# MDAnalysis/transport-analysis

Hardware: AMD Instinct MI355X
Metric: VACF lag-points/sec (n_frames x n_atoms / s) (higher is better)
Workload: dtype f64

## Files before the change

### transport_analysis_amd/csrc/wfft.hpp

```cpp
#pragma once
#include <hip/hip_runtime.h>

#include <type_traits>
#include <utility>

#include "fft_engine.hpp"

namespace ta {

#ifndef WF_NW_R0
#define WF_NW_R0 0
#define WF_NW_VAL 0
#endif

template <int LO, int HI, class F>
__device__ __forceinline__ void static_for_range(F&& f) {
    [&]<int... I>(std::integer_sequence<int, I...>) {
        (f(std::integral_constant<int, LO + I>{}), ...);
    }(std::make_integer_sequence<int, (HI > LO ? HI - LO : 0)>{});
}

typedef unsigned int wf_u32x4 __attribute__((ext_vector_type(4)));

#include "wfft_twist.inc"

template <>
struct Dft<3> {
    static __device__ __forceinline__ void run(cd (&v)[3]) {
        constexpr double kS3 = 0.86602540378443864676372317075294;
        const cd t = v[1] + v[2], d = v[1] - v[2];
        const cd m = cd{v[0].x - 0.5 * t.x, v[0].y - 0.5 * t.y};
        const cd e = cd{kS3 * d.y, -kS3 * d.x};
        v[0] = v[0] + t;
        v[1] = m + e;
        v[2] = m - e;
    }
};

template <int N>
struct DftOddTables;
template <>
struct DftOddTables<7> {
    static constexpr double c[3] = {0.62348980185873353053, -0.22252093395631440429, -0.90096886790241912624};
    static constexpr double s[3] = {0.78183148246802980871, 0.97492791218182360702, 0.43388373911755812048};
};
template <>
struct DftOddTables<9> {
    static constexpr double c[4] = {0.76604444311897803520, 0.17364817766693034885, -0.5, -0.93969262078590838405};
    static constexpr double s[4] = {0.64278760968653932632, 0.98480775301220805937, 0.86602540378443864676,
                                    0.34202014332566873304};
};
template <int N>
__device__ __forceinline__ void dft_odd(cd (&v)[N]) {
    constexpr int H = N / 2;
    using Tb = DftOddTables<N>;
    cd sp[H], dm[H];
#pragma unroll
    for (int j = 1; j <= H; ++j) {
        sp[j - 1] = v[j] + v[N - j];
        dm[j - 1] = v[j] - v[N - j];
    }
    const cd x0 = v[0];
    cd sum = x0;
#pragma unroll
    for (int j = 0; j < H; ++j) sum = sum + sp[j];
    v[0] = sum;
#pragma unroll
    for (int k = 1; k <= H; ++k) {
        double rx = x0.x, ry = x0.y, ix = 0.0, iy = 0.0;
#pragma unroll
        for (int j = 1; j <= H; ++j) {
            const int m = (j * k) % N;
            const double cm = m == 0 ? 1.0 : Tb::c[(m <= H ? m : N - m) - 1];
            const double sm = m == 0 ? 0.0 : m <= H ? Tb::s[m - 1] : -Tb::s[N - m - 1];
            rx = fma(cm, sp[j - 1].x, rx);
            ry = fma(cm, sp[j - 1].y, ry);
            ix = fma(sm, dm[j - 1].x, ix);
            iy = fma(sm, dm[j - 1].y, iy);
        }
        v[k] = cd{rx + iy, ry - ix};
        v[N - k] = cd{rx - iy, ry + ix};
    }
}
template <>
struct Dft<7> {
    static __device__ __forceinline__ void run(cd (&v)[7]) { dft_odd<7>(v); }
};
template <>
struct Dft<9> {
    static __device__ __forceinline__ void run(cd (&v)[9]) { dft_odd<9>(v); }
};

template <int N2>
__device__ __forceinline__ void dft_2x(cd (&v)[2 * N2]) {
    constexpr int N = 2 * N2;
    cd s[2][N2];
#pragma unroll
    for (int j2 = 0; j2 < N2; ++j2) {
        const cd a = v[(2 * j2) % N], b = v[(N2 + 2 * j2) % N];
        s[0][j2] = a + b;
        s[1][j2] = a - b;
    }
    Dft<N2>::run(s[0]);
    Dft<N2>::run(s[1]);
#pragma unroll
    for (int q = 0; q < N; ++q) v[q] = s[q % 2][q % N2];
}
template <>
struct Dft<14> {
    static __device__ __forceinline__ void run(cd (&v)[14]) { dft_2x<7>(v); }
};
template <>
struct Dft<18> {
    static __device__ __forceinline__ void run(cd (&v)[18]) { dft_2x<9>(v); }
};

template <>
struct Dft<6> {
    static __device__ __forceinline__ void run(cd (&v)[6]) {
        cd s[2][3];
#pragma unroll
        for (int j2 = 0; j2 < 3; ++j2) {
            const cd a = v[(2 * j2) % 6], b = v[(3 + 2 * j2) % 6];
            s[0][j2] = a + b;
            s[1][j2] = a - b;
        }
        Dft<3>::run(s[0]);
        Dft<3>::run(s[1]);
#pragma unroll
        for (int q = 0; q < 6; ++q) v[q] = s[q % 2][q % 3];
    }
};

template <>
struct Dft<12> {
    static __device__ __forceinline__ void run(cd (&v)[12]) {
        cd s[4][3];
#pragma unroll
        for (int j2 = 0; j2 < 3; ++j2) {
            cd t[4] = {v[(4 * j2) % 12], v[(3 + 4 * j2) % 12], v[(6 + 4 * j2) % 12], v[(9 + 4 * j2) % 12]};
            Dft<4>::run(t);
#pragma unroll
            for (int k1 = 0; k1 < 4; ++k1) s[k1][j2] = t[k1];
        }
#pragma unroll
        for (int k1 = 0; k1 < 4; ++k1) Dft<3>::run(s[k1]);
#pragma unroll
        for (int q = 0; q < 12; ++q) v[q] = s[q % 4][q % 3];
    }
};

template <>
struct Dft<10> {
    static __device__ __forceinline__ void run(cd (&v)[10]) {
        cd s[2][5];
#pragma unroll
        for (int j2 = 0; j2 < 5; ++j2) {
            const cd a = v[(2 * j2) % 10], b = v[(5 + 2 * j2) % 10];
            s[0][j2] = a + b;
            s[1][j2] = a - b;
        }
        Dft<5>::run(s[0]);
        Dft<5>::run(s[1]);
#pragma unroll
        for (int q = 0; q < 10; ++q) v[q] = s[q % 2][q % 5];
    }
};

template <>
struct Dft<20> {
    static __device__ __forceinline__ void run(cd (&v)[20]) {
        cd s[4][5];
#pragma unroll
        for (int j2 = 0; j2 < 5; ++j2) {
            cd t[4] = {v[(4 * j2) % 20], v[(5 + 4 * j2) % 20], v[(10 + 4 * j2) % 20], v[(15 + 4 * j2) % 20]};
            Dft<4>::run(t);
#pragma unroll
            for (int k1 = 0; k1 < 4; ++k1) s[k1][j2] = t[k1];
        }
#pragma unroll
        for (int k1 = 0; k1 < 4; ++k1) Dft<5>::run(s[k1]);
#pragma unroll
        for (int q = 0; q < 20; ++q) v[q] = s[q % 4][q % 5];
    }
};

template <int R0>
struct DftTwisted {
    static constexpr bool kHave = false;
};
template <int R0>
__device__ __forceinline__ cd wf_twist_in(const cd (&v)[R0], int n, int n2) {
    const cd x = v[n % R0];
    return ((n >= R0 ? 1 : 0) + n2) & 1 ? cd{-x.x, -x.y} : x;
}
template <>
struct DftTwisted<18> {
    static constexpr bool kHave = true;
    static __device__ __forceinline__ void run(cd (&v)[18]) {
        cd s[2][9];
#pragma unroll
        for (int j2 = 0; j2 < 9; ++j2) {
            const cd a = wf_twist_in<18>(v, 2 * j2, j2), b = wf_twist_in<18>(v, 9 + 2 * j2, j2);
            s[0][j2] = cd{a.x + b.y, a.y - b.x};
            s[1][j2] = cd{a.x - b.y, a.y + b.x};
        }
        Dft<9>::run(s[0]);
        Dft<9>::run(s[1]);
#pragma unroll
        for (int q = 0; q < 18; ++q) v[q] = s[q % 2][(q % 9 + 5) % 9];
    }
};
template <>
struct DftTwisted<20> {
    static constexpr bool kHave = true;
    static __device__ __forceinline__ void run(cd (&v)[20]) {
        cd s[4][5];
#pragma unroll
        for (int j2 = 0; j2 < 5; ++j2) {
            const cd a = wf_twist_in<20>(v, 4 * j2, j2), b = wf_twist_in<20>(v, 5 + 4 * j2, j2);
            const cd c = wf_twist_in<20>(v, 10 + 4 * j2, j2), d = wf_twist_in<20>(v, 15 + 4 * j2, j2);
            const cd p = cd{a.x + c.y, a.y - c.x}, m = cd{a.x - c.y, a.y + c.x};
            const cd e = cd{b.x + d.y, b.y - d.x}, f = cd{b.x - d.y, b.y + d.x};
            const double ex = e.x + e.y, ey = e.y - e.x;
            const double fx = f.y - f.x, fy = f.x + f.y;
            s[0][j2] = cd{fma(kR2, ex, p.x), fma(kR2, ey, p.y)};
            s[2][j2] = cd{fma(-kR2, ex, p.x), fma(-kR2, ey, p.y)};
            s[1][j2] = cd{fma(kR2, fx, m.x), fma(-kR2, fy, m.y)};
            s[3][j2] = cd{fma(-kR2, fx, m.x), fma(kR2, fy, m.y)};
        }
#pragma unroll
        for (int k1 = 0; k1 < 4; ++k1) Dft<5>::run(s[k1]);
#pragma unroll
        for (int q = 0; q < 20; ++q) v[q] = s[q % 4][(q % 5 + 3) % 5];
    }
};

constexpr int kWfStageRows = 14 + 8;
inline size_t wf_table_elems(int R0, int R) { return 2 * (size_t)R * R0 * 512 + kWfStageRows * 64; }
inline cd wf_tan_form(long num, long den) {
    const long double pi = 3.141592653589793238462643383279502884L;
    num %= den;
    if (4 * num == den) return cd{-0x1p200, 0x1p-200};
    if (4 * num == 3 * den) return cd{0x1p200, 0x1p-200};
    if (num == 0) return cd{0.0, 1.0};
    if (2 * num == den) return cd{0.0, -1.0};
    const long double h = 2.0L * pi * (long double)num / (long double)den;
    const long double c = cosl(h), sn = -sinl(h);
    return cd{(double)(sn / c), (double)c};
}
inline void wf_fill_table(int R0, int R, cd* a) {
    const long L = 2L * R * R0 * 512;
    const long double pi = 3.141592653589793238462643383279502884L;
    for (long n = 0; n < L; ++n) {
        if (n == 0) a[n] = cd{1.0, 0.0};
        else if (2 * n == L) a[n] = cd{-1.0, 0.0};
        else if (4 * n == L) a[n] = cd{0.0, -1.0};
        else if (4 * n == 3 * L) a[n] = cd{0.0, 1.0};
        else {
            const long double h = 2.0L * pi * (long double)n / (long double)L;
            a[n] = cd{(double)cosl(h), (double)-sinl(h)};
        }
    }
    for (int r = 1; r < 8; ++r)
        for (int l = 0; l < 64; ++l) {
            a[L + (r - 1) * 64 + l] = a[(L / 512) * l * r];
            a[L + (6 + r) * 64 + l] = a[(L / 64) * (l & 7) * r];
        }
    cd* t = a + L + 14 * 64;
    for (int l = 0; l < 64; ++l) {
        const long gb = 8 * (l >> 3), gc = 8 * (l & 7) + (l >> 3);
        const long g[2] = {gb, gc};
        for (int st = 0; st < 2; ++st) {
            t[(4 * st + 0) * 64 + l] = wf_tan_form(4 * g[st], 512);
            t[(4 * st + 1) * 64 + l] = wf_tan_form(2 * g[st], 512);
            t[(4 * st + 2) * 64 + l] = wf_tan_form(g[st], 512);
            t[(4 * st + 3) * 64 + l] = wf_tan_form(g[st] + 64, 512);
        }
    }
}

template <int R0_>
struct WPlan {
    static constexpr int R0 = R0_;
    static constexpr int N1 = 512;
    static constexpr int NW = R0 == WF_NW_R0 ? WF_NW_VAL : R0 <= 4 ? 2 : R0 <= 7 ? 4 : 8;
    static constexpr int NT = 64 * NW;
    static constexpr int K1 = (N1 + NT - 1) / NT;
#ifndef WF_SPREAD_ALL
    static constexpr bool kSpreadRows = R0 >= 9 && R0 <= 16;
#else
    static constexpr bool kSpreadRows = WF_SPREAD_ALL && (R0 < 18 || R0 == WF_NW_R0);
#endif
#ifndef WF_REG_EXCHANGE
    static constexpr bool kRegExchange = R0 >= 16;
#else
    static constexpr bool kRegExchange = WF_REG_EXCHANGE;
#endif
#ifndef WF_REG_EXCHANGE_SINGLE
    static constexpr bool kRegExchangeSingle = R0 == 2 || R0 == 7 || R0 == 9 || R0 == 10 || R0 == 12 || R0 == 14;
#else
    static constexpr bool kRegExchangeSingle = (WF_REG_EXCHANGE_SINGLE >> (R0 - 1)) & 1;
#endif
#ifndef WF_MINW_R0
    static __host__ __device__ constexpr int min_waves(bool , bool lng) { return R0 == 2 ? 4 : 1; }
#else
    static __host__ __device__ constexpr int min_waves(bool, bool) { return R0 == WF_MINW_R0 ? WF_MINW_VAL : 1; }
#endif
    static constexpr bool kTwResident = true;
    static constexpr int M = R0 * N1;
    static constexpr int NS1 = (R0 + NW - 1) / NW;
    static constexpr int NLO = R0 / NW, REM = R0 % NW;
    static __host__ __device__ constexpr int sub_count(int wave) { return NLO + (wave < REM ? 1 : 0); }
    static __host__ __device__ constexpr int sub_base(int wave) { return wave * NLO + (wave < REM ? wave : REM); }
    static constexpr size_t kLds = (size_t)M * sizeof(cd);

    struct RealSel {
        unsigned qmask[2];
        unsigned q1mask[2];
    };
    static __host__ __device__ constexpr int owner(int q) {
        for (int w = 0; w < NW; ++w)
            if (q >= sub_base(w) && q < sub_base(w) + sub_count(w)) return w;
        return 0;
    }
    static __host__ __device__ constexpr RealSel real_selection() {
        RealSel r{{0u, 0u}, {0u, 0u}};
        for (int t = 0; t < 2; ++t) {
            int load[8] = {0, 0, 0, 0, 0, 0, 0, 0}, simd[4] = {0, 0, 0, 0};
            auto take = [&](int q, bool self) {
                r.qmask[t] |= 1u << q;
                if (self) r.q1mask[t] |= 1u << q;
                ++load[owner(q)];
                ++simd[owner(q) % 4];
            };
            const int span = t == 0 ? R0 : R0 - 1;
            for (int q = 0; q < R0; ++q)
                if ((span - q + R0) % R0 == q) take(q, true);
            for (int q = 0; q < R0; ++q) {
                const int m = (span - q + R0) % R0;
                if (m <= q) continue;
                const int wa = owner(q), wb = owner(m);
                const int ca = 16 * load[wa] + simd[wa % 4], cb = 16 * load[wb] + simd[wb % 4];
                take(cb < ca ? m : q, false);
            }
        }
        return r;
    }
    static constexpr RealSel kRealSel = real_selection();
};

__device__ __forceinline__ cd wf_load(__amdgpu_buffer_rsrc_t r, unsigned lane_off, unsigned uni_off) {
    const wf_u32x4 v = __builtin_amdgcn_raw_buffer_load_b128(r, lane_off, uni_off, 0);
    return __builtin_bit_cast(cd, v);
}

struct WfSubPost {
    int lane, hi, lo;
    __device__ __forceinline__ explicit WfSubPost(int lane_) : lane(lane_) {
        asm volatile("" : "+v"(lane));
        hi = lane >> 3;
        lo = lane & 7;
    }
    __device__ __forceinline__ void read_a(const cd* __restrict__ reg, cd (&v)[8]) const {
#pragma unroll
        for (int n2 = 0; n2 < 8; ++n2) v[n2] = reg[64 * n2 + lane];
    }
    __device__ __forceinline__ void stage_a(cd* __restrict__ reg, cd (&v)[8], const cd (&twa)[7]) const {
        Dft<8>::run(v);
#pragma unroll
        for (int a = 1; a < 8; ++a) v[a] = cmul(v[a], twa[a - 1]);
        __builtin_amdgcn_wave_barrier();
#pragma unroll
        for (int a = 0; a < 8; ++a) reg[a * 64 + (lane ^ (8 * (a & 1)))] = v[a];
        __builtin_amdgcn_wave_barrier();
        const int base = hi * 64 + (lo ^ (8 * (hi & 1)));
#pragma unroll
        for (int n1 = 0; n1 < 8; ++n1) v[n1] = reg[base ^ (8 * n1)];
        __builtin_amdgcn_wave_barrier();
    }
    __device__ __forceinline__ void stage_b(cd* __restrict__ reg, cd (&v)[8], const cd (&twb)[7]) const {
        Dft<8>::run(v);
#pragma unroll
// ... 74 lines not shown
#pragma unroll
    for (int a = 0; a < 8; ++a)
        if (!(a & 1))
#pragma unroll
            for (int d = 0; d < 4; ++d) {
                const unsigned lo = w[a][d], hi = w[a | 1][d];
                w[a][d] = __builtin_amdgcn_update_dpp(lo, hi, 0x128, 0xF, 0xC, false);
                w[a | 1][d] = __builtin_amdgcn_update_dpp(hi, lo, 0x128, 0xF, 0x3, false);
            }
#pragma unroll
    for (int a = 0; a < 8; ++a) {
        wf_u32x4 t;
        t.x = w[a][0], t.y = w[a][1], t.z = w[a][2], t.w = w[a][3];
        v[a] = __builtin_bit_cast(cd, t);
    }
}

struct WfAddr {
    unsigned we, wo, re, ro, x16, b2w, b2r;
    __device__ __forceinline__ void init(int lane, unsigned q_bytes) {
        const int hi = lane >> 3, lo = lane & 7;
        we = q_bytes + 16u * (unsigned)lane;
        wo = q_bytes + 16u * (unsigned)(lane ^ 8);
        const unsigned rb = q_bytes + 16u * (unsigned)(hi * 64 + lo);
        re = rb + 128u * (unsigned)(hi & 1);
        ro = rb - 128u * (unsigned)(hi & 1);
        x16 = 16u * (unsigned)(hi ^ lo);
        b2w = q_bytes + 1024u * (unsigned)hi;
        b2r = b2w + 128u * (unsigned)lo;
    }
    __device__ __forceinline__ unsigned w2(int k) const { return (x16 ^ (16u * (unsigned)k)) + b2w; }
    __device__ __forceinline__ unsigned r2(int k) const { return (x16 ^ (16u * (unsigned)k)) + b2r; }
};
struct WfSub {
    const WfAddr& ad;
    unsigned char* smem;
    __device__ __forceinline__ WfSub(const WfAddr& ad_, unsigned char* smem_) : ad(ad_), smem(smem_) {}
    __device__ __forceinline__ cd& at(unsigned base, unsigned off) const {
        return *reinterpret_cast<cd*>(__builtin_assume_aligned(smem + (base + off), 16));
    }
    template <unsigned SO>
    __device__ __forceinline__ void read_a(cd (&v)[8]) const {
#pragma unroll
        for (int n2 = 0; n2 < 8; ++n2) v[n2] = at(ad.we, SO + 1024u * n2);
    }
    template <unsigned SO>
    __device__ __forceinline__ void stage_a_w(cd (&v)[8]) const {
        Dft<8>::run(v);
        __builtin_amdgcn_wave_barrier();
#pragma unroll
        for (int a = 0; a < 8; ++a) at(a & 1 ? ad.wo : ad.we, SO + 1024u * a) = v[a];
        __builtin_amdgcn_wave_barrier();
    }
    template <unsigned SO>
    __device__ __forceinline__ void stage_a_r(cd (&v)[8]) const {
        __builtin_amdgcn_wave_barrier();
#pragma unroll
        for (int n1 = 0; n1 < 8; ++n1) v[n1] = at(n1 & 1 ? ad.ro : ad.re, SO + 128u * n1);
        __builtin_amdgcn_wave_barrier();
    }
    template <unsigned SO, bool XV = false>
    __device__ __forceinline__ void stage_a(cd (&v)[8]) const {
        if constexpr (XV) {
            Dft<8>::run(v);
            wf_transpose_hi(v);
        } else {
            stage_a_w<SO>(v);
            stage_a_r<SO>(v);
        }
    }
    template <unsigned SO>
    __device__ __forceinline__ void stage_b_w(cd (&v)[8], const WfTw& tw) const {
        wf_dft8_tw(v, tw.b);
        __builtin_amdgcn_wave_barrier();
#pragma unroll
        for (int b = 0; b < 8; ++b) at(ad.w2(b), SO + 128u * b) = v[b];
        __builtin_amdgcn_wave_barrier();
    }
    template <unsigned SO>
    __device__ __forceinline__ void stage_b_r(cd (&v)[8]) const {
        __builtin_amdgcn_wave_barrier();
#pragma unroll
        for (int n0 = 0; n0 < 8; ++n0) v[n0] = at(ad.r2(n0), SO);
        __builtin_amdgcn_wave_barrier();
    }
    template <unsigned SO>
    __device__ __forceinline__ void stage_b(cd (&v)[8], const WfTw& tw) const {
        stage_b_w<SO>(v, tw);
        stage_b_r<SO>(v);
    }
    __device__ __forceinline__ void stage_c(cd (&v)[8], const WfTw& tw, double (&acc)[8]) const {
        wf_dft8_tw(v, tw.c);
#pragma unroll
        for (int c = 0; c < 8; ++c) acc[c] = fma(v[c].y, v[c].y, fma(v[c].x, v[c].x, acc[c]));
    }
    __device__ __forceinline__ void stage_c_w(cd (&v)[8], const WfTw& tw, double (&acc)[8], double wgt) const {
        wf_dft8_tw(v, tw.c);
#pragma unroll
        for (int c = 0; c < 8; ++c) acc[c] = fma(wgt, fma(v[c].y, v[c].y, v[c].x * v[c].x), acc[c]);
    }
};

constexpr unsigned kWfSubBytes = 512 * sizeof(cd);

struct WfNoHook {
    template <class T>
    __device__ __forceinline__ void operator()(T) const {}
};
template <int I>
using wf_part = std::integral_constant<int, I>;

template <int S0, bool XV = false, class Hook = WfNoHook>
__device__ __forceinline__ void wf_sub512(const WfSub& w, const WfTw& tw, double (&acc)[8], Hook&& hook = Hook{}) {
    cd v[8];
    w.read_a<S0 * kWfSubBytes>(v);
    hook(wf_part<0>{});
    w.template stage_a<S0 * kWfSubBytes, XV>(v);
    hook(wf_part<1>{});
    w.stage_b<S0 * kWfSubBytes>(v, tw);
    hook(wf_part<2>{});
    w.stage_c(v, tw, acc);
    hook(wf_part<3>{});
}

template <int S0, bool XV = false>
__device__ __forceinline__ void wf_sub512_w(const WfSub& w, const WfTw& tw, double (&acc)[8], double wgt) {
    cd v[8];
    w.read_a<S0 * kWfSubBytes>(v);
    w.template stage_a<S0 * kWfSubBytes, XV>(v);
    w.stage_b<S0 * kWfSubBytes>(v, tw);
    w.stage_c_w(v, tw, acc, wgt);
}

template <int S0, bool XV = false, class Hook = WfNoHook>
__device__ __forceinline__ void wf_sub512_x2(const WfSub& w, const WfTw& tw, double (&acc0)[8],
                                             double (&acc1)[8], Hook&& hook = Hook{}) {
    constexpr unsigned A = S0 * kWfSubBytes, B = A + kWfSubBytes;
    cd v0[8], v1[8];
    w.read_a<A>(v0);
    w.read_a<B>(v1);
    __builtin_amdgcn_wave_barrier();
    hook(wf_part<0>{});
    w.template stage_a<A>(v0);
    w.template stage_a<B, XV>(v1);
    hook(wf_part<1>{});
    w.stage_b<A>(v0, tw);
    w.stage_b<B>(v1, tw);
    hook(wf_part<2>{});
    w.stage_c(v0, tw, acc0);
    w.stage_c(v1, tw, acc1);
    hook(wf_part<3>{});
}

template <bool XV = false, class Hook = WfNoHook>
__device__ __forceinline__ void wf_sub512_x3(const WfSub& w, const WfTw& tw, double (&acc0)[8],
                                             double (&acc1)[8], double (&acc2)[8], Hook&& hook = Hook{}) {
    constexpr unsigned A = 0, B = kWfSubBytes, C = 2 * kWfSubBytes;
    cd v0[8], v1[8], v2[8];
    w.read_a<A>(v0);
    w.read_a<B>(v1);
    w.read_a<C>(v2);
    __builtin_amdgcn_wave_barrier();
    hook(wf_part<0>{});
    w.template stage_a<A>(v0);
    w.template stage_a<B>(v1);
    w.template stage_a<C, XV>(v2);
    hook(wf_part<1>{});
    w.stage_b<A>(v0, tw);
    w.stage_b<B>(v1, tw);
    w.stage_b<C>(v2, tw);
    hook(wf_part<2>{});
    w.stage_c(v0, tw, acc0);
    w.stage_c(v1, tw, acc1);
    w.stage_c(v2, tw, acc2);
    hook(wf_part<3>{});
}

__device__ __forceinline__ void wf_unit_of(long atom, int k, int D, long* pair, int* kind) {
    const long c0 = atom * D;
    if (D == 2) {
        *pair = atom, *kind = 2;
    } else if (D == 1) {
        *pair = c0 >> 1, *kind = (int)(c0 & 1);
    } else if ((c0 & 1) == 0) {
        *pair = (c0 >> 1) + k, *kind = k == 0 ? 2 : 0;
    } else {
        *pair = (c0 >> 1) + k, *kind = k == 0 ? 1 : 2;
    }
}

typedef unsigned int wf_u32x2 __attribute__((__vector_size__(2 * sizeof(unsigned int))));

__device__ __forceinline__ cd wf_cfma(cd acc, cd a, cd b) {
    return {acc.x + (a.x * b.x - a.y * b.y), acc.y + (a.x * b.y + a.y * b.x)};
}

template <bool S, class A, class B>
__device__ __forceinline__ auto& wf_pick(A& a, B& b) {
    if constexpr (S) return a;
    else return b;
}

#ifndef WF_PASS_SPLIT
#define WF_PASS_SPLIT 1
#endif
#ifndef WF_SEED_DERIVE
#define WF_SEED_DERIVE 2
#endif
#ifndef WF_TWIST_FOLD
#define WF_TWIST_FOLD 1
#endif
#ifndef WF_TWIDDLE_MIRROR
#define WF_TWIDDLE_MIRROR 1
#endif
template <class P, bool BYP, bool LONG, bool SRC32>
constexpr bool wf_pass_split = WF_PASS_SPLIT && !BYP && !LONG && !SRC32 && (P::R0 == 18 || P::R0 == 20);

__device__ __forceinline__ cd wf_csqr(cd a) { return {a.x * a.x - a.y * a.y, 2.0 * (a.x * a.y)}; }

template <class P, bool BYP, bool LONG, bool STAMP, bool SRC32, int PASS>
__device__ __forceinline__ void wf_accum_body(unsigned char* smem_raw, const double* __restrict__ pm, long pitch, int T,
                                              long n_units, const cd* __restrict__ tw2, double* __restrict__ accg, int D,
                                              int R_arg, unsigned long long* __restrict__ stamps) {
    cd* lds = reinterpret_cast<cd*>(smem_raw);
    constexpr int R0 = P::R0, N1 = P::N1, NW = P::NW, NS1 = P::NS1, M = P::M;
    static_assert(!(SRC32 && LONG), "float32 slabs: plans without an outer radix only");
    static_assert(PASS < 0 || (!BYP && !LONG), "a compile-time pass: lag sums without an outer radix");
    const int R = LONG ? R_arg : 1, npass = 2 * R, L = npass * M;
    const int tid = threadIdx.x, wave = tid >> 6;
    int lane = tid & 63;
    const int bi = blockIdx.x >> 3;
    const int pass = PASS >= 0 ? PASS : bi % npass;
    constexpr bool kTwistFold = PASS == 1 && WF_TWIST_FOLD && DftTwisted<R0>::kHave;
    constexpr bool kMirror = PASS >= 0 && WF_TWIDDLE_MIRROR && R0 % 2 == 0;
    const long tuple = (blockIdx.x & 7) + 8 * (bi / npass), n_tuples = gridDim.x / npass;
    const int upa = BYP ? (D == 3 ? 2 : 1) : 1;
    const int grp = BYP && (D & 1) ? 2 : 1;

    double acc[NS1][8];
#pragma unroll
    for (int s = 0; s < NS1; ++s)
#pragma unroll
        for (int c = 0; c < 8; ++c) acc[s][c] = 0.0;
    unsigned long long st_acc[4] = {0, 0, 0, 0}, st_prev = 0, st_t0 = 0, st_r0 = 0, st_tail = 0, st_s2end = 0;
    if constexpr (STAMP) {
        st_prev = st_t0 = __builtin_amdgcn_s_memtime();
        st_r0 = __builtin_amdgcn_s_memrealtime();
    }
#define WF_STAMP(i)                                                   \
    if constexpr (STAMP) {                                            \
        const unsigned long long now_ = __builtin_amdgcn_s_memtime(); \
        st_acc[i] += now_ - st_prev;                                  \
        st_prev = now_;                                               \
    }
    const __amdgpu_buffer_rsrc_t twr =
        __builtin_amdgcn_make_buffer_rsrc(const_cast<cd*>(tw2), 0, (L + kWfStageRows * 64) * 16, 0x00020000);
    auto unit_rsrc = [&](long item, int k, int* kind) {
        long pair = item;
        const bool live = item < n_units;
        *kind = 2;
        if constexpr (BYP) wf_unit_of(live ? item : 0, k, D, &pair, kind);
        if constexpr (SRC32)
            return __builtin_amdgcn_make_buffer_rsrc(
                const_cast<float*>(reinterpret_cast<const float*>(pm) + (live ? pair : 0) * pitch * 2), 0,
                live ? T * 8 : 0, 0x00020000);
        else
            return __builtin_amdgcn_make_buffer_rsrc(const_cast<double*>(pm + (live ? pair : 0) * pitch * 2), 0,
                                                     live ? T * 16 : 0, 0x00020000);
    };
    using RowT = std::conditional_t<SRC32, wf_u32x2, cd>;
    auto load_row = [&](__amdgpu_buffer_rsrc_t rs, int kd, int u, unsigned row_off) -> RowT {
        if constexpr (SRC32) {
            return __builtin_amdgcn_raw_buffer_load_b64(rs, (unsigned)u * 8u, row_off * 8u, 0);
        } else {
            if (!BYP || kd == 2) return wf_load(rs, (unsigned)u * 16u, row_off * 16u);
            return cd{__builtin_bit_cast(double, __builtin_amdgcn_raw_buffer_load_b64(
                                                     rs, (unsigned)u * 16u + (unsigned)kd * 8u, row_off * 16u, 0)),
                      0.0};
        }
    };
    [[maybe_unused]] auto wf_widen = [&](wf_u32x2 r, int kd) {
        if (!BYP || kd == 2)
            return cd{(double)__builtin_bit_cast(float, (unsigned)r[0]), (double)__builtin_bit_cast(float, (unsigned)r[1])};
        return cd{(double)__builtin_bit_cast(float, (unsigned)(kd ? r[1] : r[0])), 0.0};
    };
    constexpr int K1 = P::K1, NT = P::NT;
    RowT xx[K1][R0];
    auto issue_loads = [&](__amdgpu_buffer_rsrc_t rs, int kd) {
#pragma unroll
        for (int k1 = 0; k1 < K1; ++k1) {
            const int u = tid + NT * k1;
            if (K1 * NT != N1 && u >= N1) continue;
            if (!BYP || kd == 2) {
#pragma unroll
                for (int j = 0; j < R0; ++j) xx[k1][j] = load_row(rs, 2, u, (unsigned)(N1 * j));
            } else {
#pragma unroll
                for (int j = 0; j < R0; ++j) xx[k1][j] = load_row(rs, kd, u, (unsigned)(N1 * j));
            }
        }
    };
#ifndef WF_LOAD_PARTS
#define WF_LOAD_PARTS 4
#endif
    constexpr int NR = K1 * R0;
    constexpr bool kSpread = P::kSpreadRows || (SRC32 && R0 >= 18);
#ifndef WF_SPREAD32_TAIL
#define WF_SPREAD32_TAIL 0
#endif
    constexpr int NSPREAD = WF_LOAD_PARTS != 4 ? 0 : (kSpread ? (SRC32 && R0 >= 18 ? NR - WF_SPREAD32_TAIL : NR) : 0);
    auto issue_row = [&](auto ii, __amdgpu_buffer_rsrc_t rs, int kd) {
        constexpr int i = decltype(ii)::value, k1 = i / R0, j = i % R0;
        const int u = tid + NT * k1;
        if (K1 * NT != N1 && u >= N1) return;
        if (!BYP || kd == 2) xx[k1][j] = load_row(rs, 2, u, (unsigned)(N1 * j));
        else xx[k1][j] = load_row(rs, kd, u, (unsigned)(N1 * j));
    };
    auto issue_loads_part = [&](auto part_c, __amdgpu_buffer_rsrc_t rs, int kd) {
        constexpr int PART = decltype(part_c)::value;
        static_for_range<PART * NSPREAD / 4, (PART + 1) * NSPREAD / 4>([&](auto ii) { issue_row(ii, rs, kd); });
    };
    auto issue_loads_tail = [&](__amdgpu_buffer_rsrc_t rs, int kd) {
        static_for_range<NSPREAD, NR>([&](auto ii) { issue_row(ii, rs, kd); });
    };
    int kind = 2, nkind = 2;
    __amdgpu_buffer_rsrc_t crs = unit_rsrc(tuple * grp, 0, &kind);
    issue_loads(crs, kind);
    WfTw stw;
    auto load_stage_tw = [&]() {
#pragma unroll
        for (int a = 0; a < 4; ++a) {
            stw.b[a] = wf_load(twr, (unsigned)lane * 16u, (unsigned)(L + (14 + a) * 64) * 16u);
            stw.c[a] = wf_load(twr, (unsigned)lane * 16u, (unsigned)(L + (18 + a) * 64) * 16u);
        }
    };
    constexpr bool kTwRes = P::kTwResident && !(BYP && LONG && R0 >= 18);
    if constexpr (kTwRes) load_stage_tw();
    WfAddr wad;
    wad.init(lane, (unsigned)P::sub_base(wave) * kWfSubBytes);
    const WfSub wsub(wad, smem_raw);
    int k = 0;
    bool zero_pending = false;
    for (long item = tuple * grp; item < n_units;) {
#ifndef WF_REAL_S1_SKIP
#define WF_REAL_S1_SKIP 0
#endif
        const unsigned qsel = (WF_REAL_S1_SKIP && BYP && kind != 2) ? P::kRealSel.qmask[pass ? 1 : 0] : ~0u;
#pragma unroll
        for (int k1 = 0; k1 < K1; ++k1) {
        const int u = tid + NT * k1;
        if (K1 * NT != N1 && u >= N1) continue;
        [[maybe_unused]] cd xwide[SRC32 ? R0 : 1];
        if constexpr (SRC32) {
#pragma unroll
            for (int j = 0; j < R0; ++j) xwide[j] = wf_widen(xx[k1][j], kind);
        }
        cd(&x)[R0] = wf_pick<SRC32>(xwide, xx[k1]);
        cd g, g2, h;
        auto load_seeds = [&]() {
            if constexpr (PASS == 1 && WF_SEED_DERIVE >= 1) {
                h = wf_load(twr, (unsigned)u * 16u, 0u);
                g = wf_csqr(h);
            } else {
                g = wf_load(twr, (unsigned)(u * R) * 32u, 0u);
                if (PASS != 0) h = wf_load(twr, (unsigned)(u * pass) * 16u, 0u);
            }
            if constexpr ((PASS == 0 && WF_SEED_DERIVE >= 2) || (PASS == 1 && WF_SEED_DERIVE >= 3)) g2 = wf_csqr(g);
            else g2 = wf_load(twr, (unsigned)(u * R) * 64u, 0u);
        };
        if constexpr (!LONG) load_seeds();
        if constexpr (LONG) {
            const int sj = pass * N1, so = pass * M;
            if (pass) {
                int idx = 0;
#pragma unroll
                for (int j = 1; j < R0; ++j) {
                    idx += sj;
                    idx -= idx >= L ? L : 0;
                    x[j] = cmul(x[j], tw_uniform(tw2, idx));
                }
            }
            auto outer_rows = [&](auto single) {
                int base = 0;
                for (int jo = 1; jo < R; ++jo) {
                    base += so;
                    base -= base >= L ? L : 0;
                    if (jo * M >= T) break;
                    int idx = base;
                    constexpr int NZ = 10;
#pragma unroll
                    for (int j0 = 0; j0 < R0; j0 += NZ) {
                        cd z[NZ];
#pragma unroll
                        for (int i = 0; i < NZ; ++i)
                            if (j0 + i < R0)
                                z[i] = load_row(crs, decltype(single)::value ? kind : 2, u, (unsigned)(N1 * (j0 + i) + M * jo));
#pragma unroll
                        for (int i = 0; i < NZ; ++i)
                            if (j0 + i < R0) {
                                x[j0 + i] = wf_cfma(x[j0 + i], z[i], tw_uniform(tw2, idx));
                                idx += sj;
                                idx -= idx >= L ? L : 0;
                            }
                        __builtin_amdgcn_sched_barrier(0);
                    }
                }
            };
            if (BYP && kind != 2) outer_rows(std::true_type{});
            else outer_rows(std::false_type{});
            __builtin_amdgcn_sched_barrier(0);
            load_seeds();
        } else if (pass) {
            if constexpr (!kTwistFold) {
#pragma unroll
                for (int j = 1; j < R0; ++j) x[j] = cmul(x[j], cd{WfTwist<R0>::re(j), WfTwist<R0>::im(j)});
            }
        }
        if constexpr (kTwistFold) DftTwisted<R0>::run(x);
        else Dft<R0>::run(x);
        if constexpr (kMirror) {
            constexpr int H = R0 / 2;
            cd te, to;
            if constexpr (PASS == 0) {
                te = g2;
                to = g;
                lds[u] = x[0];
#pragma unroll
                for (int q = 1; q <= H; ++q) {
                    if (q >= 3 && (q & 1)) to = cmul(to, g2);
                    else if (q >= 3) te = cmul(te, g2);
                    const cd t = (q & 1) ? to : te;
                    x[q] = cmul(x[q], t);
                    lds[q * N1 + u] = x[q];
                    if (q < H) {
                        x[R0 - q] = cmulc(x[R0 - q], t);
                        lds[(R0 - q) * N1 + u] = x[R0 - q];
                    }
                }
            } else {
                te = h;
                to = cmul(h, g);
#pragma unroll
                for (int q = 0; q < H; ++q) {
                    if (q >= 2 && (q & 1)) to = cmul(to, g2);
                    else if (q >= 2) te = cmul(te, g2);
                    const cd t = (q & 1) ? to : te;
                    x[q] = cmul(x[q], t);
                    lds[q * N1 + u] = x[q];
                    x[R0 - 1 - q] = cmulc(x[R0 - 1 - q], t);
                    lds[(R0 - 1 - q) * N1 + u] = x[R0 - 1 - q];
                }
            }
        } else {
            cd te, to;
            if constexpr (PASS == 0) {
                te = cd{1.0, 0.0};
                to = g;
            } else {
                te = pass ? h : cd{1.0, 0.0};
                to = pass ? cmul(h, g) : g;
                if (pass) x[0] = cmul(x[0], te);
            }
            if (!(WF_REAL_S1_SKIP && BYP) || (qsel & 1u)) lds[u] = x[0];
            if constexpr (R0 > 1) {
                x[1] = cmul(x[1], to);
                if (!(WF_REAL_S1_SKIP && BYP) || (qsel & 2u)) lds[N1 + u] = x[1];
            }
#pragma unroll
            for (int q = 2; q < R0; ++q) {
                if (q & 1) {
                    to = cmul(to, g2);
                    x[q] = cmul(x[q], to);
                } else {
                    te = (PASS == 0 && q == 2) ? g2 : cmul(te, g2);
                    x[q] = cmul(x[q], te);
                }
                if (!(WF_REAL_S1_SKIP && BYP) || (qsel >> q & 1u)) lds[q * N1 + u] = x[q];
            }
        }
        }
        if constexpr (!kTwRes) {
            asm volatile("" : "+v"(lane));
            load_stage_tw();
        }
        WF_STAMP(0)
        __syncthreads();
        if (BYP && zero_pending) {
#pragma unroll
            for (int s = 0; s < NS1; ++s)
#pragma unroll
                for (int c = 0; c < 8; ++c) acc[s][c] = 0.0;
            zero_pending = false;
        }
        const bool last_of_item = !BYP || k == upa - 1;
        long nitem = item;
        if (last_of_item) {
            if (BYP && grp == 2 && (item & 1) == 0 && item + 1 < n_units) nitem = item + 1;
            else nitem = (item & ~(long)(grp - 1)) + grp * n_tuples;
        }
        const int nk = last_of_item ? 0 : k + 1;
        const __amdgpu_buffer_rsrc_t nrs = unit_rsrc(nitem, nk, &nkind);
        auto row_hook = [&](auto part_c) {
#if WF_LOAD_PARTS == 4
            issue_loads_part(part_c, nrs, nkind);
#endif
        };
        if (BYP && kind != 2) {
            const int wv = __builtin_amdgcn_readfirstlane(wave);
            static_for_range<0, 4>([&](auto part_c) { row_hook(part_c); });
            const unsigned qs = P::kRealSel.qmask[pass ? 1 : 0] >> P::sub_base(wv);
            const unsigned q1 = P::kRealSel.q1mask[pass ? 1 : 0] >> P::sub_base(wv);
            static_for_range<0, NS1>([&](auto ss) {
                constexpr int s = decltype(ss)::value;
                if ((s < P::NLO || wv < P::REM) && (qs >> s & 1u))
                    wf_sub512_w<s, P::kRegExchangeSingle>(wsub, stw, acc[s], (q1 >> s & 1u) ? 1.0 : 2.0);
            });
        } else
        if constexpr (NS1 == 3 && P::NLO == 2 && P::REM != 0) {
            if constexpr (SRC32) {
                if (wave < P::REM) wf_sub512_x3<P::kRegExchange>(wsub, stw, acc[0], acc[1], acc[2], row_hook);
                else wf_sub512_x2<0, P::kRegExchange>(wsub, stw, acc[0], acc[1], row_hook);
            } else {
                if (wave < P::REM) wf_sub512_x3<P::kRegExchange>(wsub, stw, acc[0], acc[1], acc[2]);
                else wf_sub512_x2<0, P::kRegExchange>(wsub, stw, acc[0], acc[1]);
            }
        } else {
            static_for_range<0, NS1>([&](auto ss) {
                constexpr int s = decltype(ss)::value;
                constexpr bool full = s < P::NLO;
                constexpr bool nfull = s + 1 < P::NLO;
                constexpr bool head = full && nfull && (s % 2 == 0);
                constexpr bool tail = full && s > 0 && (s % 2 == 1);
                if constexpr (head) {
                    if constexpr (s == 0) wf_sub512_x2<s, P::kRegExchange>(wsub, stw, acc[s], acc[s + 1], row_hook);
                    else wf_sub512_x2<s, P::kRegExchange>(wsub, stw, acc[s], acc[s + 1]);
                } else if constexpr (!tail) {
                    if constexpr (s == 0) wf_sub512<s, P::kRegExchangeSingle>(wsub, stw, acc[s], row_hook);
                    else if (full || wave < P::REM) wf_sub512<s, P::kRegExchangeSingle>(wsub, stw, acc[s]);
                }
            });
        }
        if constexpr (STAMP) st_s2end = __builtin_amdgcn_s_memtime();
        const int wv = __builtin_amdgcn_readfirstlane(wave);
        auto store_acc = [&](long row) {
            const __amdgpu_buffer_rsrc_t sr = __builtin_amdgcn_make_buffer_rsrc(
                accg + (row * npass + pass) * (long)M, 0, M * 8, 0x00020000);
#pragma unroll
            for (int s = 0; s < NS1; ++s) {
                const int q = P::sub_base(wv) + s;
                if (s < P::NLO || wv < P::REM) {
#pragma unroll
                    for (int c2 = 0; c2 < 4; ++c2) {
                        const cd two{acc[s][2 * c2], acc[s][2 * c2 + 1]};
                        __builtin_amdgcn_raw_buffer_store_b128(__builtin_bit_cast(wf_u32x4, two), sr, (unsigned)lane * 16u,
                                                               (unsigned)((q * 4 + c2) * 64) * 16u, 0);
                    }
                }
            }
        };
        if constexpr (BYP) {
            if (last_of_item) {
                store_acc(item);
                zero_pending = true;
            }
        } else {
            if constexpr (!kMirror)
                if (nitem >= n_units) store_acc(tuple);
        }
        __builtin_amdgcn_sched_barrier(0);
        issue_loads_tail(nrs, nkind);
        kind = nkind, item = nitem, k = nk, crs = nrs;
        if constexpr (STAMP) st_tail += __builtin_amdgcn_s_memtime() - st_s2end;
        WF_STAMP(1)
        __syncthreads();
    }
    if constexpr (kMirror) {
        if (tuple * grp < n_units) {
            const int wv = __builtin_amdgcn_readfirstlane(wave);
            const __amdgpu_buffer_rsrc_t sr = __builtin_amdgcn_make_buffer_rsrc(
                accg + (tuple * npass + pass) * (long)M, 0, M * 8, 0x00020000);
            int ln = (int)__builtin_amdgcn_mbcnt_hi(~0u, __builtin_amdgcn_mbcnt_lo(~0u, 0u));
            asm volatile("" : "+v"(ln));
            const unsigned lm = (unsigned)(ln >= 8 ? ln - 8 : ln ? ln + 55 : 63) * 16u;
#pragma unroll
            for (int s = 0; s < NS1; ++s) {
                const int q = P::sub_base(wv) + s;
                if (s < P::NLO || wv < P::REM) {
                    const bool mir = PASS == 0 ? q > R0 / 2 : q >= R0 / 2;
                    const bool carry = mir && ln == 0;
                    const unsigned ld = mir ? lm : (unsigned)ln * 16u;
                    const unsigned v0 = ld + (carry ? 3080u : 0u);
                    const unsigned ve = ld + (carry ? 8u : 1024u);
                    const unsigned vo = ld + (carry ? 0u : 8u);
#pragma unroll
                    for (int cc = 0; cc < 8; ++cc) {
                        const unsigned at = (unsigned)((cc >> 1) * 64 * 16 + (cc & 1) * 8);
                        __builtin_amdgcn_raw_buffer_store_b64(__builtin_bit_cast(wf_u32x2, acc[s][cc]), sr,
                                                              cc == 0 ? v0 : (cc & 1) ? vo + (at - 8u) : ve + (at - 1024u),
                                                              (unsigned)(q * 4 * 64) * 16u, 0);
                    }
                }
            }
        }
    }
    if constexpr (!BYP) {
        if (tuple * grp >= n_units) {
            const int wv = __builtin_amdgcn_readfirstlane(wave);
            const __amdgpu_buffer_rsrc_t sr = __builtin_amdgcn_make_buffer_rsrc(
                accg + (tuple * npass + pass) * (long)M, 0, M * 8, 0x00020000);
#pragma unroll
            for (int s = 0; s < NS1; ++s) {
                const int q = P::sub_base(wv) + s;
                if (s < P::sub_count(wv)) {
#pragma unroll
                    for (int c2 = 0; c2 < 4; ++c2)
                        __builtin_amdgcn_raw_buffer_store_b128(__builtin_bit_cast(wf_u32x4, cd{0.0, 0.0}), sr,
                                                               (unsigned)lane * 16u, (unsigned)((q * 4 + c2) * 64) * 16u, 0);
                }
            }
        }
    }
    if constexpr (STAMP) {
        st_acc[2] = __builtin_amdgcn_s_memtime() - st_t0;
        st_acc[3] = __builtin_amdgcn_s_memrealtime() - st_r0;
        if (lane == 0 && (wave == 0 || wave == NW / 2)) {
            for (int i = 0; i < 4; ++i) stamps[16 * (long)blockIdx.x + (wave ? 4 : 0) + i] = st_acc[i];
            stamps[16 * (long)blockIdx.x + 8 + (wave ? 1 : 0)] = st_tail;
        }
    }
#undef WF_STAMP
}

template <class P, bool BYP = false, bool LONG = false, bool STAMP = false, bool SRC32 = false>
__global__ void __launch_bounds__(P::NT, P::min_waves(BYP, LONG))
    k_wsplit_accum(const double* __restrict__ pm, long pitch, int T, long n_units,
                   const cd* __restrict__ tw2, double* __restrict__ accg, int D, int R_arg,
                   unsigned long long* __restrict__ stamps) {
    extern __shared__ __attribute__((aligned(16))) unsigned char smem_raw[];
    if constexpr (wf_pass_split<P, BYP, LONG, SRC32>) {
#ifdef WF_FIX_PASS
        wf_accum_body<P, BYP, LONG, STAMP, SRC32, WF_FIX_PASS>(smem_raw, pm, pitch, T, n_units, tw2, accg, D, R_arg, stamps);
        return;
#endif
        if ((blockIdx.x >> 3) & 1)
            wf_accum_body<P, BYP, LONG, STAMP, SRC32, 1>(smem_raw, pm, pitch, T, n_units, tw2, accg, D, R_arg, stamps);
        else
            wf_accum_body<P, BYP, LONG, STAMP, SRC32, 0>(smem_raw, pm, pitch, T, n_units, tw2, accg, D, R_arg, stamps);
    } else {
        wf_accum_body<P, BYP, LONG, STAMP, SRC32, -1>(smem_raw, pm, pitch, T, n_units, tw2, accg, D, R_arg, stamps);
    }
}

struct WfSubT {
    int lane, hi, lo;
    __device__ __forceinline__ explicit WfSubT(int lane_) : lane(lane_) {
        asm volatile("" : "+v"(lane));
        hi = lane >> 3;
        lo = lane & 7;
    }
    __device__ __forceinline__ void run(cd* __restrict__ reg, cd (&v)[8], const cd (&twa)[7],
                                        const cd (&twb)[7]) const {
        Dft<8>::run(v);
#pragma unroll
        for (int n0 = 1; n0 < 8; ++n0) v[n0] = cmul(v[n0], twb[n0 - 1]);
        __builtin_amdgcn_wave_barrier();
        const int x = lo ^ hi;
#pragma unroll
        for (int n0 = 0; n0 < 8; ++n0) reg[(hi * 8 + n0) * 8 + (x ^ n0)] = v[n0];
        __builtin_amdgcn_wave_barrier();
#pragma unroll
        for (int b = 0; b < 8; ++b) v[b] = reg[lane * 8 + (b ^ x)];
        __builtin_amdgcn_wave_barrier();
        Dft<8>::run(v);
        __builtin_amdgcn_wave_barrier();
        const int base = hi * 64 + (lo ^ (8 * (hi & 1)));
#pragma unroll
        for (int n1 = 0; n1 < 8; ++n1) reg[base ^ (8 * n1)] = v[n1];
        __builtin_amdgcn_wave_barrier();
#pragma unroll
        for (int a = 0; a < 8; ++a) v[a] = reg[a * 64 + (lane ^ (8 * (a & 1)))];
        __builtin_amdgcn_wave_barrier();
#pragma unroll
        for (int a = 1; a < 8; ++a) v[a] = cmul(v[a], twa[a - 1]);
        Dft<8>::run(v);
        __builtin_amdgcn_wave_barrier();
#pragma unroll
        for (int n2 = 0; n2 < 8; ++n2) reg[64 * n2 + lane] = v[n2];
        __builtin_amdgcn_wave_barrier();
    }
};



template <class P, bool LONG = false, int PF = 0>
__global__ void __launch_bounds__(P::NT)
    k_winverse(const double* __restrict__ spec, int T, long n_items, const cd* __restrict__ tw2,
               double* __restrict__ out, long ld, int R_arg) {
    extern __shared__ __attribute__((aligned(16))) unsigned char smem_raw[];
    cd* lds = reinterpret_cast<cd*>(smem_raw);
    constexpr int R0 = P::R0, N1 = P::N1, NW = P::NW, NT = P::NT, K1 = P::K1, M = P::M, NSA = P::NS1;
    static_assert(!LONG || PF == 0, "the spectrum prefetch is for the single-transform case");
    static_assert(PF <= NSA, "prefetch depth counts sub-series of a wave");
    const int R = LONG ? R_arg : 1, L = 2 * R * M;
    int tid = threadIdx.x, lane = tid & 63;
    const int wave = tid >> 6;
    const __amdgpu_buffer_rsrc_t twr =
        __builtin_amdgcn_make_buffer_rsrc(const_cast<cd*>(tw2), 0, (L + kWfStageRows * 64) * 16, 0x00020000);
    cd v[NSA][8];
    auto load_spec = [&](long item, int cp, int s) {
        const int wv = __builtin_amdgcn_readfirstlane(wave);
        const int q = wv + NW * s;
        const bool live = item < n_items && q < R0;
        const __amdgpu_buffer_rsrc_t sr = __builtin_amdgcn_make_buffer_rsrc(
            const_cast<double*>(spec + (live ? item : 0) * (long)L + (long)(2 * cp) * M), 0, live ? 2 * M * 8 : 0,
            0x00020000);
#pragma unroll
        for (int c2 = 0; c2 < 4; ++c2) {
            const cd a = wf_load(sr, (unsigned)lane * 16u, (unsigned)((q * 4 + c2) * 64) * 16u);
            const cd b = wf_load(sr, (unsigned)lane * 16u, (unsigned)(M / 2 + (q * 4 + c2) * 64) * 16u);
            v[s][2 * c2] = cd{a.x, b.x};
            v[s][2 * c2 + 1] = cd{a.y, b.y};
        }
    };
    constexpr bool kHoistNorm = !LONG && R0 >= 9;
    double rnorm[kHoistNorm ? K1 : 1][kHoistNorm ? R0 : 1];
    if constexpr (kHoistNorm) {
#pragma unroll
        for (int k1 = 0; k1 < K1; ++k1)
#pragma unroll
            for (int j = 0; j < R0; ++j) {
                const int n = tid + NT * k1 + N1 * j;
                rnorm[k1][j] = n < T ? 1.0 / (2.0 * (double)M * (double)(T - n)) : 0.0;
            }
    }
#pragma unroll
    for (int s = 0; s < PF; ++s) load_spec(blockIdx.x, 0, s);
    for (long item = blockIdx.x; item < n_items; item += gridDim.x) {
        for (int cp = 0; cp < R; ++cp) {
            asm volatile("" : "+v"(tid), "+v"(lane));
            {
                cd twa[7], twb[7];
#pragma unroll
                for (int a = 0; a < 7; ++a) {
                    twa[a] = wf_load(twr, (unsigned)lane * 16u, (unsigned)(L + a * 64) * 16u);
                    twb[a] = wf_load(twr, (unsigned)lane * 16u, (unsigned)(L + (7 + a) * 64) * 16u);
                }
#pragma unroll
                for (int s = PF; s < NSA; ++s) load_spec(item, cp, s);
                const WfSubT wt(lane);
#pragma unroll
                for (int s = 0; s < NSA; ++s) {
                    const int q = wave + NW * s;
                    if (NW * s + NW - 1 < R0 || q < R0) wt.run(lds + q * N1, v[s], twa, twb);
                }
            }
            __syncthreads();
            if constexpr (PF > 0) {
                __builtin_amdgcn_sched_barrier(0);
#pragma unroll
                for (int s = 0; s < PF; ++s) load_spec(item + gridDim.x, 0, s);
                __builtin_amdgcn_sched_barrier(0);
            }
            cd xx[K1][R0];
#pragma unroll
            for (int k1 = 0; k1 < K1; ++k1) {
                const int u = tid + NT * k1;
                if (K1 * NT != N1 && u >= N1) continue;
                cd(&x)[R0] = xx[k1];
                const cd g = wf_load(twr, (unsigned)(u * R) * 32u, 0u), g2 = wf_load(twr, (unsigned)(u * R) * 64u, 0u);
#pragma unroll
                for (int q = 0; q < R0; ++q) x[q] = lds[q * N1 + u];
                cd te = cd{1.0, 0.0}, to = g;
                if constexpr (R0 > 1) x[1] = cmul(x[1], to);
#pragma unroll
                for (int q = 2; q < R0; ++q) {
                    if (q & 1) {
                        to = cmul(to, g2);
                        x[q] = cmul(x[q], to);
                    } else {
                        te = cmul(te, g2);
// ... 287 lines not shown
```

Before: 118.8 billion.

## Reorder row loads to match first DFT layer and fence the layer schedule

With WF_ROW_ORDER on by default, rows are loaded in the order the first radix-2 or radix-4 layer of the R0=18/20 DFT consumes them. Sched barriers after each group of rows and first-layer butterflies let compute start as data arrives and keep register pressure down. Twiddle-seed derivation moves after the DFT so it does not lengthen the critical path. An optional, off-by-default mode issues part of the next item's loads in the middle of the three-subFFT stage, and a stamp records first-layer timing. The added fences constrain the compiler scheduler and could serialize work it would otherwise interleave.

```diff
diff --git a/transport_analysis_amd/csrc/wfft.hpp b/transport_analysis_amd/csrc/wfft.hpp
--- a/transport_analysis_amd/csrc/wfft.hpp
+++ b/transport_analysis_amd/csrc/wfft.hpp
@@ -91,8 +91,26 @@
     static __device__ __forceinline__ void run(cd (&v)[9]) { dft_odd<9>(v); }
 };
 
-template <int N2>
-__device__ __forceinline__ void dft_2x(cd (&v)[2 * N2]) {
+struct WfNoMid {
+    __device__ __forceinline__ void operator()() const {}
+};
+template <int R0>
+constexpr int kWfRowGroup = R0 == 20 ? 4 : 6;
+template <int R0>
+constexpr int wf_row_at(int i) {
+    return R0 == 20 ? (5 * (i % 4) + 4 * (i / 4)) % 20 : (9 * (i % 2) + 2 * (i / 2)) % 18;
+}
+template <bool ORD>
+__device__ __forceinline__ void wf_step_fence() {
+    if constexpr (ORD) __builtin_amdgcn_sched_barrier(0);
+}
+template <bool ORD>
+__device__ __forceinline__ void wf_step_tie(cd& a, cd& b) {
+    if constexpr (ORD) asm volatile("" : "+v"(a.x), "+v"(a.y), "+v"(b.x), "+v"(b.y));
+}
+
+template <int N2, bool ORD = false, class F = WfNoMid>
+__device__ __forceinline__ void dft_2x(cd (&v)[2 * N2], F&& mid = F{}) {
     constexpr int N = 2 * N2;
     cd s[2][N2];
 #pragma unroll
@@ -100,7 +118,10 @@
         const cd a = v[(2 * j2) % N], b = v[(N2 + 2 * j2) % N];
         s[0][j2] = a + b;
         s[1][j2] = a - b;
-    }
+        wf_step_tie<ORD>(s[0][j2], s[1][j2]);
+        if (j2 % 3 == 2) wf_step_fence<ORD>();
+    }
+    mid();
     Dft<N2>::run(s[0]);
     Dft<N2>::run(s[1]);
 #pragma unroll
@@ -112,7 +133,10 @@
 };
 template <>
 struct Dft<18> {
-    static __device__ __forceinline__ void run(cd (&v)[18]) { dft_2x<9>(v); }
+    template <bool ORD = false, class F = WfNoMid>
+    static __device__ __forceinline__ void run(cd (&v)[18], F&& mid = F{}) {
+        dft_2x<9, ORD>(v, mid);
+    }
 };
 
 template <>
@@ -169,7 +193,8 @@
 
 template <>
 struct Dft<20> {
-    static __device__ __forceinline__ void run(cd (&v)[20]) {
+    template <bool ORD = false, class F = WfNoMid>
+    static __device__ __forceinline__ void run(cd (&v)[20], F&& mid = F{}) {
         cd s[4][5];
 #pragma unroll
         for (int j2 = 0; j2 < 5; ++j2) {
@@ -177,7 +202,9 @@
             Dft<4>::run(t);
 #pragma unroll
             for (int k1 = 0; k1 < 4; ++k1) s[k1][j2] = t[k1];
-        }
+            wf_step_fence<ORD>();
+        }
+        mid();
 #pragma unroll
         for (int k1 = 0; k1 < 4; ++k1) Dft<5>::run(s[k1]);
 #pragma unroll
@@ -197,14 +224,18 @@
 template <>
 struct DftTwisted<18> {
     static constexpr bool kHave = true;
-    static __device__ __forceinline__ void run(cd (&v)[18]) {
+    template <bool ORD = false, class F = WfNoMid>
+    static __device__ __forceinline__ void run(cd (&v)[18], F&& mid = F{}) {
         cd s[2][9];
 #pragma unroll
         for (int j2 = 0; j2 < 9; ++j2) {
             const cd a = wf_twist_in<18>(v, 2 * j2, j2), b = wf_twist_in<18>(v, 9 + 2 * j2, j2);
             s[0][j2] = cd{a.x + b.y, a.y - b.x};
             s[1][j2] = cd{a.x - b.y, a.y + b.x};
-        }
+            wf_step_tie<ORD>(s[0][j2], s[1][j2]);
+            if (j2 % 3 == 2) wf_step_fence<ORD>();
+        }
+        mid();
         Dft<9>::run(s[0]);
         Dft<9>::run(s[1]);
 #pragma unroll
@@ -214,7 +245,8 @@
 template <>
 struct DftTwisted<20> {
     static constexpr bool kHave = true;
-    static __device__ __forceinline__ void run(cd (&v)[20]) {
+    template <bool ORD = false, class F = WfNoMid>
+    static __device__ __forceinline__ void run(cd (&v)[20], F&& mid = F{}) {
         cd s[4][5];
 #pragma unroll
         for (int j2 = 0; j2 < 5; ++j2) {
@@ -228,7 +260,9 @@
             s[2][j2] = cd{fma(-kR2, ex, p.x), fma(-kR2, ey, p.y)};
             s[1][j2] = cd{fma(kR2, fx, m.x), fma(-kR2, fy, m.y)};
             s[3][j2] = cd{fma(-kR2, fx, m.x), fma(kR2, fy, m.y)};
-        }
+            wf_step_fence<ORD>();
+        }
+        mid();
 #pragma unroll
         for (int k1 = 0; k1 < 4; ++k1) Dft<5>::run(s[k1]);
 #pragma unroll
@@ -609,9 +643,9 @@
     hook(wf_part<3>{});
 }
 
-template <bool XV = false, class Hook = WfNoHook>
-__device__ __forceinline__ void wf_sub512_x3(const WfSub& w, const WfTw& tw, double (&acc0)[8],
-                                             double (&acc1)[8], double (&acc2)[8], Hook&& hook = Hook{}) {
+template <bool XV = false, class Hook = WfNoHook, class Early = WfNoMid>
+__device__ __forceinline__ void wf_sub512_x3(const WfSub& w, const WfTw& tw, double (&acc0)[8], double (&acc1)[8],
+                                             double (&acc2)[8], Hook&& hook = Hook{}, Early&& early = Early{}) {
     constexpr unsigned A = 0, B = kWfSubBytes, C = 2 * kWfSubBytes;
     cd v0[8], v1[8], v2[8];
     w.read_a<A>(v0);
@@ -629,6 +663,10 @@
     hook(wf_part<2>{});
     w.stage_c(v0, tw, acc0);
     w.stage_c(v1, tw, acc1);
+    constexpr bool kEarly = !std::is_same_v<std::remove_cvref_t<Early>, WfNoMid>;
+    wf_step_fence<kEarly>();
+    early();
+    wf_step_fence<kEarly>();
     w.stage_c(v2, tw, acc2);
     hook(wf_part<3>{});
 }
@@ -669,6 +707,15 @@
 #endif
 #ifndef WF_TWIDDLE_MIRROR
 #define WF_TWIDDLE_MIRROR 1
+#endif
+#ifndef WF_ROW_ORDER
+#define WF_ROW_ORDER 1
+#endif
+#ifndef WF_X3_EARLY
+#define WF_X3_EARLY 0
+#endif
+#ifndef WF_X3_EARLY_ROWS
+#define WF_X3_EARLY_ROWS 8
 #endif
 template <class P, bool BYP, bool LONG, bool SRC32>
 constexpr bool wf_pass_split = WF_PASS_SPLIT && !BYP && !LONG && !SRC32 && (P::R0 == 18 || P::R0 == 20);
@@ -690,6 +737,8 @@
     const int pass = PASS >= 0 ? PASS : bi % npass;
     constexpr bool kTwistFold = PASS == 1 && WF_TWIST_FOLD && DftTwisted<R0>::kHave;
     constexpr bool kMirror = PASS >= 0 && WF_TWIDDLE_MIRROR && R0 % 2 == 0;
+    constexpr bool kRowOrder = PASS >= 0 && WF_ROW_ORDER && (R0 == 18 || R0 == 20);
+    constexpr bool kX3Early = PASS >= 0 && WF_X3_EARLY && P::NS1 == 3 && P::NLO == 2 && P::REM != 0;
     const long tuple = (blockIdx.x & 7) + 8 * (bi / npass), n_tuples = gridDim.x / npass;
     const int upa = BYP ? (D == 3 ? 2 : 1) : 1;
     const int grp = BYP && (D & 1) ? 2 : 1;
@@ -700,6 +749,7 @@
 #pragma unroll
         for (int c = 0; c < 8; ++c) acc[s][c] = 0.0;
     unsigned long long st_acc[4] = {0, 0, 0, 0}, st_prev = 0, st_t0 = 0, st_r0 = 0, st_tail = 0, st_s2end = 0;
+    [[maybe_unused]] unsigned long long st_layer1 = 0;
     if constexpr (STAMP) {
         st_prev = st_t0 = __builtin_amdgcn_s_memtime();
         st_r0 = __builtin_amdgcn_s_memrealtime();
@@ -767,11 +817,13 @@
 #endif
     constexpr int NSPREAD = WF_LOAD_PARTS != 4 ? 0 : (kSpread ? (SRC32 && R0 >= 18 ? NR - WF_SPREAD32_TAIL : NR) : 0);
     auto issue_row = [&](auto ii, __amdgpu_buffer_rsrc_t rs, int kd) {
-        constexpr int i = decltype(ii)::value, k1 = i / R0, j = i % R0;
+        constexpr int i = decltype(ii)::value, k1 = i / R0;
+        constexpr int j = kRowOrder ? wf_row_at<R0>(i % R0) : i % R0;
         const int u = tid + NT * k1;
         if (K1 * NT != N1 && u >= N1) return;
         if (!BYP || kd == 2) xx[k1][j] = load_row(rs, 2, u, (unsigned)(N1 * j));
         else xx[k1][j] = load_row(rs, kd, u, (unsigned)(N1 * j));
+        if constexpr (kRowOrder) wf_step_fence<(i % R0 + 1) % kWfRowGroup<R0> == 0>();
     };
     auto issue_loads_part = [&](auto part_c, __amdgpu_buffer_rsrc_t rs, int kd) {
         constexpr int PART = decltype(part_c)::value;
@@ -780,9 +832,17 @@
     auto issue_loads_tail = [&](__amdgpu_buffer_rsrc_t rs, int kd) {
         static_for_range<NSPREAD, NR>([&](auto ii) { issue_row(ii, rs, kd); });
     };
+    constexpr int NEARLY = kX3Early ? (WF_X3_EARLY_ROWS < NR ? WF_X3_EARLY_ROWS : NR) : 0;
+    auto issue_loads_early = [&](__amdgpu_buffer_rsrc_t rs, int kd) {
+        static_for_range<0, NEARLY>([&](auto ii) { issue_row(ii, rs, kd); });
+    };
+    auto issue_loads_late = [&](__amdgpu_buffer_rsrc_t rs, int kd) {
+        static_for_range<NEARLY, NR>([&](auto ii) { issue_row(ii, rs, kd); });
+    };
     int kind = 2, nkind = 2;
     __amdgpu_buffer_rsrc_t crs = unit_rsrc(tuple * grp, 0, &kind);
-    issue_loads(crs, kind);
+    if constexpr (kRowOrder) static_for_range<0, NR>([&](auto ii) { issue_row(ii, crs, kind); });
+    else issue_loads(crs, kind);
     WfTw stw;
     auto load_stage_tw = [&]() {
 #pragma unroll
@@ -814,16 +874,20 @@
         }
         cd(&x)[R0] = wf_pick<SRC32>(xwide, xx[k1]);
         cd g, g2, h;
+        auto derive_seeds = [&]() {
+            if constexpr (PASS == 1 && WF_SEED_DERIVE >= 1) g = wf_csqr(h);
+            if constexpr ((PASS == 0 && WF_SEED_DERIVE >= 2) || (PASS == 1 && WF_SEED_DERIVE >= 3)) g2 = wf_csqr(g);
+        };
         auto load_seeds = [&]() {
             if constexpr (PASS == 1 && WF_SEED_DERIVE >= 1) {
                 h = wf_load(twr, (unsigned)u * 16u, 0u);
-                g = wf_csqr(h);
             } else {
                 g = wf_load(twr, (unsigned)(u * R) * 32u, 0u);
                 if (PASS != 0) h = wf_load(twr, (unsigned)(u * pass) * 16u, 0u);
             }
-            if constexpr ((PASS == 0 && WF_SEED_DERIVE >= 2) || (PASS == 1 && WF_SEED_DERIVE >= 3)) g2 = wf_csqr(g);
-            else g2 = wf_load(twr, (unsigned)(u * R) * 64u, 0u);
+            if constexpr (!((PASS == 0 && WF_SEED_DERIVE >= 2) || (PASS == 1 && WF_SEED_DERIVE >= 3)))
+                g2 = wf_load(twr, (unsigned)(u * R) * 64u, 0u);
+            if constexpr (!kRowOrder) derive_seeds();
         };
         if constexpr (!LONG) load_seeds();
         if constexpr (LONG) {
@@ -873,8 +937,19 @@
                 for (int j = 1; j < R0; ++j) x[j] = cmul(x[j], cd{WfTwist<R0>::re(j), WfTwist<R0>::im(j)});
             }
         }
-        if constexpr (kTwistFold) DftTwisted<R0>::run(x);
-        else Dft<R0>::run(x);
+        if constexpr (kRowOrder) {
+            auto layer1 = [&]() {
+                if constexpr (STAMP) st_layer1 += __builtin_amdgcn_s_memtime() - st_prev;
+            };
+            if constexpr (kTwistFold) DftTwisted<R0>::template run<true>(x, layer1);
+            else Dft<R0>::template run<true>(x, layer1);
+            cd& seed = wf_pick<PASS == 1 && WF_SEED_DERIVE >= 1>(h, g);
+            asm volatile("" : "+v"(seed.x), "+v"(seed.y));
+            derive_seeds();
+        } else {
+            if constexpr (kTwistFold) DftTwisted<R0>::run(x);
+            else Dft<R0>::run(x);
+        }
         if constexpr (kMirror) {
             constexpr int H = R0 / 2;
             cd te, to;
@@ -977,6 +1052,11 @@
             if constexpr (SRC32) {
                 if (wave < P::REM) wf_sub512_x3<P::kRegExchange>(wsub, stw, acc[0], acc[1], acc[2], row_hook);
                 else wf_sub512_x2<0, P::kRegExchange>(wsub, stw, acc[0], acc[1], row_hook);
+            } else if constexpr (kX3Early) {
+                if (wave < P::REM)
+                    wf_sub512_x3<P::kRegExchange>(wsub, stw, acc[0], acc[1], acc[2], WfNoHook{},
+                                                  [&]() { issue_loads_early(nrs, nkind); });
+                else wf_sub512_x2<0, P::kRegExchange>(wsub, stw, acc[0], acc[1]);
             } else {
                 if (wave < P::REM) wf_sub512_x3<P::kRegExchange>(wsub, stw, acc[0], acc[1], acc[2]);
                 else wf_sub512_x2<0, P::kRegExchange>(wsub, stw, acc[0], acc[1]);
@@ -1025,7 +1105,12 @@
                 if (nitem >= n_units) store_acc(tuple);
         }
         __builtin_amdgcn_sched_barrier(0);
-        issue_loads_tail(nrs, nkind);
+        if constexpr (kX3Early) {
+            if (wave >= P::REM) issue_loads_early(nrs, nkind);
+            issue_loads_late(nrs, nkind);
+        } else {
+            issue_loads_tail(nrs, nkind);
+        }
         kind = nkind, item = nitem, k = nk, crs = nrs;
         if constexpr (STAMP) st_tail += __builtin_amdgcn_s_memtime() - st_s2end;
         WF_STAMP(1)
@@ -1083,6 +1168,7 @@
         if (lane == 0 && (wave == 0 || wave == NW / 2)) {
             for (int i = 0; i < 4; ++i) stamps[16 * (long)blockIdx.x + (wave ? 4 : 0) + i] = st_acc[i];
             stamps[16 * (long)blockIdx.x + 8 + (wave ? 1 : 0)] = st_tail;
+            stamps[16 * (long)blockIdx.x + 10 + (wave ? 1 : 0)] = st_layer1;
         }
     }
 #undef WF_STAMP
```

Result: no change. 119.8 billion, median of 6 (+0.9%).
